# mikwieczorek/centroids-reid

Hardware: AMD Instinct MI355X
Metric: train_images_per_sec (higher is better)
Workload: dtype bf16; 1 GPU; ResNet50 256x128 CTL training step: fwd+bwd, centroid-triplet + center + xent, Adam + center SGD (BASELINE configs[1]); P=16, K=4, global_batch=64, num_classes=751, parallelism=single

## Files before the change

### centroids-reid_amd/_lib.py

```python
from __future__ import annotations

import ctypes as C
import os

import torch

_HERE = os.path.dirname(os.path.abspath(__file__))
LIB_PATH = os.environ.get("CREID_LIB_PATH") or os.path.join(_HERE, "lib", "libcreid_hip.so")

F32, BF16, F16 = 0, 1, 2
_DT = {torch.float32: F32, torch.bfloat16: BF16, torch.float16: F16}
BF16X3 = 3
EVAL_PRECISIONS = ("bf16x3",)
TRAIN_PRECISIONS = ("bf16x3",)

_lib = None

_p, _i64, _i32, _f32, _sz = C.c_void_p, C.c_int64, C.c_int32, C.c_float, C.c_size_t

SIGNATURES = {
    "creid_abi_version": (C.c_int, []),
    "creid_l2norm_rows": (C.c_int, [_p, _p, _p, _i64, _i64, C.c_int, _f32, _p]),
    "creid_row_sqnorm": (C.c_int, [_p, _p, _i64, _i64, C.c_int, _p]),
    "creid_sqdist_matrix": (C.c_int, [_p, _p, _p, _p, _i64, _i64, _i64, C.c_int, _p, _i64, _p]),
# ... 33 lines not shown
    "creid_ctl_heads_fused": (C.c_int, [_p, _p]),
    "creid_ctl_step_stats_rows": (C.c_int, [_p, _p, _i64, _i64, _i64, _p, _p, _p, _p]),
    "creid_center_loss_fwd_masked": (C.c_int, [_p, _p, _p, _p, _i64, _i64, _i64, _p, _p, _p]),
    "creid_center_loss_bwd_masked": (C.c_int, [_p, _p, _p, _p, _p, _i64, _i64, _p, _f32, _p, _p, _p]),
    "creid_xent_ls_masked": (C.c_int, [_p, _p, _p, _i64, _i64, _f32, _f32, _p, _p, _p, _p]),
    "creid_bn1d_fwd_masked": (C.c_int, [_p, _p, _i64, _i64, _p, _p, _p, _p, _f32, _f32, _p, _p, _p, _p]),
    "creid_bn1d_bwd_masked": (C.c_int, [_p, _p, _p, _i64, _i64, _p, _p, _p, _p, _p, _p, _p]),
    "creid_triplet_fwd": (C.c_int, [_p, _p, _p, _i64, _i64, _f32, _p, _p, _p, _p, _p, _p, _p, _p]),
    "creid_triplet_bwd": (C.c_int, [_p, _i64, _i64, _p, _p, _p, _p, _p, _p, _f32, _p, _p]),
    "creid_triplet_fwd_batched": (C.c_int, [_p, _p, _p, _i64, _i64, _i64, _f32, _p, _p, _p, _p, _p, _p, _p, _p]),
    "creid_triplet_bwd_batched": (C.c_int, [_p, _i64, _i64, _i64, _p, _p, _p, _p, _p, _p, _f32, _p, _p]),
    "creid_triplet_cosine_fwd": (C.c_int, [_p, _p, _p, _i64, _i64, _f32, _p, _p, _p, _p, _p, _p, _p, _p]),
    "creid_triplet_cosine_bwd": (C.c_int, [_p, _i64, _i64, _p, _p, _p, _p, _p, _p, _f32, _p, _p]),
    "creid_rownorm_fwd": (C.c_int, [_p, _i64, _i64, C.c_int, _f32, _p, _p, _p]),
    "creid_rownorm_bwd": (C.c_int, [_p, _p, _p, _i64, _i64, C.c_int, _f32, _p, _p]),
    "creid_hard_mine_from_dist": (C.c_int, [_p, _p, _i64, _p, _p, _p, _p, _p]),
    "creid_clamp_sqrt_inplace": (C.c_int, [_p, _i64, _f32, _p]),
    "creid_center_loss_fwd": (C.c_int, [_p, _p, _p, _i64, _i64, _i64, _p, _p, _p]),
    "creid_center_loss_bwd": (C.c_int, [_p, _p, _p, _p, _i64, _i64, _p, _f32, _p, _p, _p]),
    "creid_xent_ls": (C.c_int, [_p, _p, _i64, _i64, _f32, _f32, _p, _p, _p, _p]),
    "creid_bn1d_fwd": (C.c_int, [_p, _i64, _i64, _p, _p, _p, _p, C.c_int, _f32, _f32, _p, _p, _p, _p]),
    "creid_bn1d_bwd": (C.c_int, [_p, _p, _i64, _i64, _p, _p, _p, _p, _p, _p, _p]),
    "creid_gather_mean_rows": (C.c_int, [_p, _p, _p, _i64, _i64, _p, _p]),
    "creid_adam_step": (C.c_int, [_p, _p, _p, _p, _i64, _f32, _f32, _f32, _f32, _f32, _i64, _f32, _p]),
    "creid_adam_step_dev": (C.c_int, [_p, _p, _p, _p, _i64, _p, _f32, _f32, _f32, _f32, _f32, _p]),
    "creid_sgd_scaled_step": (C.c_int, [_p, _p, _i64, _f32, _f32, _p]),
    "creid_amp_scale": (C.c_int, [_p, _i64, _p, _p, _p]),
    "creid_amp_unscale_check": (C.c_int, [_p, _i64, _p, _p, _p]),
    "creid_amp_update": (C.c_int, [_p, _p, _f32, _f32, C.c_int32, _p]),
    "creid_adam_step_dev_amp": (C.c_int, [_p, _p, _p, _p, _i64, _p, _f32, _f32, _f32, _f32, _f32, _p, _p]),
    "creid_sgd_scaled_step_amp": (C.c_int, [_p, _p, _i64, _f32, _f32, _p, _p]),
    "creid_conv2d_bn_partial_rows": (_i64, [_p]),
    "creid_igemm_halo_launches": (_i64, []),
    "creid_conv2d_fwd_nhwc": (C.c_int, [_p, _p, _p, _p, _p, C.c_int, _p]),
    "creid_conv2d_fwd_affine_nhwc": (C.c_int, [_p, _p, _p, _p, _p, _p, C.c_int, C.c_int, _p]),
    "creid_conv1x1_bnrelu_fwd": (C.c_int, [_p, _p, _p, _i64, _i64, _i64, _p, _p, _p, _p, C.c_int, _p]),
    "creid_bn2d_fold_entry_bytes": (_i64, []),
    "creid_bn2d_fold_multi": (C.c_int, [_p, _i64, _p]),
    "creid_stem_conv_fwd_affine": (C.c_int, [_i64, _i64, _i64, _p, _p, _p, _p, C.c_int, C.c_int, _p]),
    "creid_stem_conv_pool_fwd_affine": (C.c_int, [_i64, _i64, _i64, _p, _p, _p, _p, C.c_int, C.c_int, _p]),
    "creid_bottleneck_c3_c1_fwd_affine": (C.c_int, [_i64, _i64, _i64, _i64, _p, _p, _p, _p, _p, _p, _p, _p, C.c_int, _p]),
    "creid_bottleneck_c3_c1_fwd_stats": (C.c_int, [_i64, _i64, _i64, _i64, _p, _p, _p, _p, _p, _p, _p, _p, C.c_int, _p]),
    "creid_conv2d_dgrad_nhwc": (C.c_int, [_p, _p, _p, _p, _p, C.c_int, _p]),
    "creid_conv2d_wgrad_workspace_bytes": (_sz, [_p, C.c_int]),
    "creid_conv2d_wgrad_nhwc": (C.c_int, [_p, _p, _p, _p, C.c_int, _p, _sz, C.c_int, _p]),
    "creid_conv2d_wgrad_partials": (C.c_int, [_p, _p, _p, _p, _sz, C.c_int, _p]),
    "creid_conv2d_wgrad_partials_bnfin": (C.c_int, [_p, _p, _p, _p, _sz, C.c_int, _p, _i64, _i64, _i64, _p, _p, _p, _p, _p, _p, _p]),
    "creid_conv2d_wgrad_reduce": (C.c_int, [_p, _p, C.c_int, _p, _sz, C.c_int, _p]),
    "creid_bn2d_bwd_finalize_wred": (C.c_int, [_p, _i64, _i64, _i64, _p, _p, _p, _p, _p, _p, _p, _p, C.c_int, _p, _sz, C.c_int, _p]),
    "creid_conv2d_wgrad_reduce_job": (C.c_int, [_p, _p, C.c_int, _p, _sz, C.c_int, _p]),
    "creid_conv2d_dgrad_x3_nhwc": (C.c_int, [_p, _p, _p, _p, _p, _p]),
    "creid_conv2d_wgrad_x3_workspace_bytes": (_sz, [_p]),
    "creid_conv2d_wgrad_x3_nhwc": (C.c_int, [_p, _p, _p, _p, C.c_int, _p, _sz, _p]),
    "creid_conv2d_wgrad_x3_partials": (C.c_int, [_p, _p, _p, _p, _sz, _p]),
    "creid_weight_prep_x3_train_multi": (C.c_int, [_p, _p, _i64, _i64, _p]),
    "creid_stem_conv_fwd": (C.c_int, [_i64, _i64, _i64, _p, _p, _p, _p, C.c_int, _p]),
    "creid_stem_conv_wgrad_workspace_bytes": (_sz, [_i64, _i64, _i64, C.c_int]),
    "creid_stem_conv_wgrad": (C.c_int, [_i64, _i64, _i64, _p, _p, _p, C.c_int, _p, _sz, C.c_int, _p]),
    "creid_image_to_nhwc4_pad": (C.c_int, [_p, _i64, _i64, _i64, C.c_int, _p, _p]),
    "creid_augment_u8": (C.c_int, [_p, _p, _i64, _i64, _i64, _i64] + [C.c_float] * 9 + [C.c_int32, C.c_int32, _p, _p]),
    "creid_resize_u8": (C.c_int, [_p, _i64, _p, _p, _p, _i64, _p, _i64, _i64, _i64, _p, _p]),
    "creid_weight_prep": (C.c_int, [_p, _i64, _i64, _i64, _i64, C.c_int, _p, _p, _p]),
    "creid_weight_prep_entry_bytes": (_i64, []),
    "creid_weight_prep_multi": (C.c_int, [_p, _p, _i64, _i64, C.c_int, _p]),
    "creid_stem_weight_prep": (C.c_int, [_p, C.c_int, _p, _p]),
    "creid_bn2d_finalize": (C.c_int, [_p, _i64, _i64, _i64, _p, _p, C.c_int, _f32, _f32, _p, _p, _p, _p, _p, _p]),
# ... 125 lines not shown
```

### centroids-reid_amd/csrc/bn_fin.hpp

```cpp
#pragma once
#include "common.hpp"

struct BnBwdFinJob {
  const float* partial;
  int rows, C;
  float inv_count;
  const float* mean;
  const float* invstd;
  const float* gamma;
  float* sums;
  float* dgamma;
  float* dbeta;
  int nblocks;
  int cw;
};

template <int NT, int CW>
__device__ __forceinline__ void bn_bwd_finalize_block_cw(const BnBwdFinJob& j, int block, void* lds) {
  constexpr int RG = NT / CW, NW = NT / 64;
  double* red = reinterpret_cast<double*>(lds);
  const int tid = threadIdx.x, cl = tid % CW, rg = tid / CW;
  const int c = block * CW + cl, C = j.C;
  double s1 = 0.0, s2 = 0.0;
  if (c < C) {
    int r = rg;
    for (; r + 3 * RG < j.rows; r += 4 * RG) {
      const float a0 = j.partial[((int64_t)r * 2) * C + c], b0 = j.partial[((int64_t)r * 2 + 1) * C + c];
      const float a1 = j.partial[((int64_t)(r + RG) * 2) * C + c], b1 = j.partial[((int64_t)(r + RG) * 2 + 1) * C + c];
      const float a2 = j.partial[((int64_t)(r + 2 * RG) * 2) * C + c], b2 = j.partial[((int64_t)(r + 2 * RG) * 2 + 1) * C + c];
      const float a3 = j.partial[((int64_t)(r + 3 * RG) * 2) * C + c], b3 = j.partial[((int64_t)(r + 3 * RG) * 2 + 1) * C + c];
      s1 += ((double)a0 + (double)a1) + ((double)a2 + (double)a3);
      s2 += ((double)b0 + (double)b1) + ((double)b2 + (double)b3);
    }
    for (; r < j.rows; r += RG) {
      s1 += (double)j.partial[((int64_t)r * 2) * C + c];
      s2 += (double)j.partial[((int64_t)r * 2 + 1) * C + c];
    }
  }
#pragma unroll
  for (int o = CW; o < 64; o <<= 1) { s1 += __shfl_xor(s1, o, 64); s2 += __shfl_xor(s2, o, 64); }
  if ((tid & 63) < CW) { red[((tid >> 6) * 2 + 0) * CW + cl] = s1; red[((tid >> 6) * 2 + 1) * CW + cl] = s2; }
  float p_mu = 0.f, p_is = 0.f, p_g = 1.f, p_db = 0.f, p_dg = 0.f;
  if (rg == 0 && c < C) {
    p_mu = j.mean[c]; p_is = j.invstd[c];
    if (j.gamma) p_g = j.gamma[c];
    if (j.dbeta) p_db = j.dbeta[c];
    if (j.dgamma) p_dg = j.dgamma[c];
  }
  __syncthreads();
  if (rg == 0 && c < C) {
    s1 = 0.0; s2 = 0.0;
#pragma unroll
    for (int q = 0; q < NW; ++q) { s1 += red[(q * 2 + 0) * CW + cl]; s2 += red[(q * 2 + 1) * CW + cl]; }
    const float invM = j.inv_count;
    const float mu = p_mu, is = p_is, k1 = p_g * is;
    const float a1 = (float)s1 * invM, a2 = (float)s2 * invM;
    j.sums[c] = k1;
    j.sums[C + c] = -k1 * is * a2;
    j.sums[2 * C + c] = -k1 * a1 + k1 * is * a2 * mu;
    if (j.dbeta) j.dbeta[c] = p_db + (float)s1;
    if (j.dgamma) j.dgamma[c] = p_dg + (float)s2;
  }
}

template <int NT>
__device__ __forceinline__ void bn_bwd_finalize_block(const BnBwdFinJob& j, int block, void* lds) {
  if (j.cw == 4) bn_bwd_finalize_block_cw<NT, 4>(j, block, lds);
  else bn_bwd_finalize_block_cw<NT, 16>(j, block, lds);
}

static inline void bn_bwd_fin_shape(BnBwdFinJob& j) {
  j.cw = (j.C <= 256 && j.rows >= 512) ? 4 : 16;
  j.nblocks = (j.C + j.cw - 1) / j.cw;
}
```

### centroids-reid_amd/csrc/conv_wgrad.hip

```cpp
#include "conv_common.hpp"
#include "wgrad_reduce.hpp"
#include "bn_fin.hpp"
#include "tune.hpp"
#include <stdlib.h>

namespace {
constexpr int WKS = 64;
constexpr int WKF = 16;
}

template <int OFF_HI>
__device__ __forceinline__ void tr_load4(const unsigned short* p, s16x4& f0lo, s16x4& f0hi, s16x4& f1lo, s16x4& f1hi) {
  const unsigned addr = (unsigned)(uintptr_t)p;
  asm volatile(
      "ds_read_b64_tr_b16 %0, %4\n\t"
      "ds_read_b64_tr_b16 %1, %4 offset:%5\n\t"
      "ds_read_b64_tr_b16 %2, %4 offset:64\n\t"
      "ds_read_b64_tr_b16 %3, %4 offset:%6"
      : "=&v"(f0lo), "=&v"(f0hi), "=&v"(f1lo), "=&v"(f1hi)
      : "v"(addr), "i"(OFF_HI), "i"(OFF_HI + 64)
      : "memory");
}
__device__ __forceinline__ void tr_wait8(s16x4& a, s16x4& b, s16x4& c, s16x4& d, s16x4& e, s16x4& f, s16x4& g, s16x4& h) {
  asm volatile("s_waitcnt lgkmcnt(0)" : "+v"(a), "+v"(b), "+v"(c), "+v"(d), "+v"(e), "+v"(f), "+v"(g), "+v"(h)::"memory");
}

template <int NW>
__device__ __forceinline__ void tr_wait8_n(s16x4& a, s16x4& b, s16x4& c, s16x4& d, s16x4& e, s16x4& f, s16x4& g, s16x4& h) {
  asm volatile("s_waitcnt lgkmcnt(%8)" : "+v"(a), "+v"(b), "+v"(c), "+v"(d), "+v"(e), "+v"(f), "+v"(g), "+v"(h) : "n"(NW) : "memory");
}

template <int NW, int IM, int JN>
__device__ __forceinline__ void tr_wait_set(s16x4 (&al)[IM], s16x4 (&ah)[IM], s16x4 (&bl)[JN], s16x4 (&bh)[JN]) {
  if constexpr (IM == 2 && JN == 2)
    asm volatile("s_waitcnt lgkmcnt(%8)" : "+v"(al[0]), "+v"(ah[0]), "+v"(al[1]), "+v"(ah[1]), "+v"(bl[0]), "+v"(bh[0]), "+v"(bl[1]), "+v"(bh[1]) : "n"(NW) : "memory");
  else if constexpr (IM == 2 && JN == 1)
    asm volatile("s_waitcnt lgkmcnt(%6)" : "+v"(al[0]), "+v"(ah[0]), "+v"(al[1]), "+v"(ah[1]), "+v"(bl[0]), "+v"(bh[0]) : "n"(NW) : "memory");
// ... 382 lines not shown
    float* ex = reinterpret_cast<float*>(smem_all);
    const int t256 = tid & 255;
    if (kg == 1) {
#pragma unroll
      for (int i = 0; i < IM; ++i)
#pragma unroll
        for (int j = 0; j < JN; ++j)
#pragma unroll
          for (int r = 0; r < 16; ++r) ex[((i * JN + j) * 16 + r) * 256 + t256] = acc[i][j][r];
    }
    __syncthreads();
    if (kg == 1) return;
#pragma unroll
    for (int i = 0; i < IM; ++i)
#pragma unroll
      for (int j = 0; j < JN; ++j)
#pragma unroll
        for (int r = 0; r < 16; ++r) acc[i][j][r] += ex[((i * JN + j) * 16 + r) * 256 + t256];
  }
  const int l31 = lane & 31, kh = lane >> 5;
  float* wsp = ws + (int64_t)split * NCO * g.K;
#pragma unroll
  for (int i = 0; i < IM; ++i)
#pragma unroll
    for (int j = 0; j < JN; ++j)
#pragma unroll
      for (int r = 0; r < 16; ++r) {
        const int co = co0 + wm * (TM / 2) + i * 32 + (r & 3) + 8 * (r >> 2) + 4 * kh;
        const int kc = k0 + wn * (TN / 2) + j * 32 + l31;
        wsp[(int64_t)co * g.K + kc] = acc[i][j][r];
      }
}

template <int TM, int TN>
__global__ __launch_bounds__(256) void wgrad_f32_kernel(IGemmGeom g, const float* __restrict__ dy,
                                                        const float* __restrict__ x, int NCO, float* __restrict__ ws,
                                                        int tiles_k, int m_per_split) {
  constexpr int IM = TM / 64, JN = TN / 64;
  constexpr int CA = TM / 4, CB = TN / 4;
  constexpr int RA = 256 / CA, RB = 256 / CB;
  constexpr int NA = (WKF + RA - 1) / RA, NBL = (WKF + RB - 1) / RB;
  __shared__ __attribute__((aligned(16))) float Ad[WKF][TM];
  __shared__ __attribute__((aligned(16))) float Bx[WKF][TN];
  const int tid = threadIdx.x, lane = tid & 63, wave = tid >> 6;
  const int wm = wave >> 1, wn = wave & 1;
  const int tile = blockIdx.x, split = blockIdx.y;
  const int tile_co = tile / tiles_k, tile_k = tile - tile_co * tiles_k;
  const int co0 = tile_co * TM, k0 = tile_k * TN;
  const int m_begin = split * m_per_split, m_end = min(g.M, m_begin + m_per_split);
  const int span_mask = (1 << g.log2span) - 1;
  const int a_ch = tid % CA, a_row = tid / CA;
  const int b_ch = tid % CB, b_row = tid / CB;
  const int kcol = k0 + 4 * b_ch;
  const int tap = kcol >> g.log2span, cc = kcol & span_mask;
  const int tr = tap / g.kw, ts = tap - tr * g.kw;
  float4 ra[NA], rb[NBL];
  auto gload = [&](int mb) {
#pragma unroll
    for (int i = 0; i < NA; ++i) {
      const int pr = a_row + RA * i, m = mb + pr;
      ra[i] = (pr < WKF && m < m_end) ? *reinterpret_cast<const float4*>(dy + (int64_t)m * NCO + co0 + 4 * a_ch)
                                      : make_float4(0.f, 0.f, 0.f, 0.f);
    }
#pragma unroll
    for (int i = 0; i < NBL; ++i) {
      const int pr = b_row + RB * i, m = mb + pr;
// ... 230 lines not shown
  for (int e = 0; e < 4; ++e) {
    const int kc = kc0 + e;
    const int tap = kc >> log2span, within = kc & span_mask;
    const int r = tap / kw_taps, s = tap % kw_taps + within / cpitch, c = within % cpitch;
    if (r < kh && s < kw && c < cin) {
      float* dst = dw_oihw + (((int64_t)co * cin + c) * kh + r) * kw + s;
      *dst = accumulate ? *dst + v[e] : v[e];
    }
  }
}

__global__ __launch_bounds__(256) void wgrad_reduce_taps_kernel(const float* __restrict__ ws, int splits, int NCO, int K,
                                                                int cin, int taps, float* __restrict__ dw_oihw,
                                                                int accumulate) {
  extern __shared__ float tr_lds[];
  const int co = blockIdx.x;
  const int64_t total = (int64_t)NCO * K;
  const float* src = ws + (int64_t)co * K;
  for (int e = threadIdx.x; e < K; e += 256) {
    float a0 = 0.f, a1 = 0.f;
    int sp = 0;
    for (; sp + 1 < splits; sp += 2) { a0 += src[(int64_t)sp * total + e]; a1 += src[(int64_t)(sp + 1) * total + e]; }
    if (sp < splits) a0 += src[(int64_t)sp * total + e];
    const int tap = e / cin, c = e - tap * cin;
    tr_lds[c * taps + tap] = a0 + a1;
  }
  __syncthreads();
  float* dst = dw_oihw + (int64_t)co * K;
  for (int e = threadIdx.x; e < K; e += 256) dst[e] = accumulate ? dst[e] + tr_lds[e] : tr_lds[e];
}

static int ilog2x(int64_t v) { int l = 0; while ((1LL << l) < v) ++l; return ((1LL << l) == v) ? l : -1; }

struct WgradPlan { int tm, tn, tiles, tiles_k, splits, m_per_split, xcd, stages, ws, kg; };

static WgradPlan plan_wgrad(int M, int NCO, int K, int dtype, int stride = 1) {
  static const int target = [] { const char* e = getenv("CREID_WGRAD_TARGET_WGS"); int v = e ? atoi(e) : 0; return v > 0 ? v : 512; }();
  static const int max_splits_pref = [] { const char* e = getenv("CREID_WGRAD_MAX_SPLITS"); int v = e ? atoi(e) : 0; return v > 0 ? v : (1 << 30); }();
  const int ks = creid_is16(dtype) ? WKS : WKF;
  const int cand[3][2] = {{128, 128}, {128, 64}, {64, 64}};
  WgradPlan p;
  p.stages = 0; p.ws = 0; p.kg = 0;
  TunePlan tp;
  const bool have_plan = creid_is16(dtype) && creid_tune_lookup(CREID_TUNE_WGRAD, M, NCO, K, stride << 1, tp);
  if (have_plan && !((tp.p0 == 64 || tp.p0 == 128) && (tp.p1 == 64 || tp.p1 == 128) && NCO % tp.p0 == 0 && K % tp.p1 == 0 && tp.p2 >= 1))
    creid_tune_declined(CREID_TUNE_WGRAD, M, NCO, K, stride << 1);
  else if (have_plan) {
    p.tm = tp.p0; p.tn = tp.p1;
    p.stages = (tp.p2 >> 16) & 15; p.ws = (tp.p2 >> 20) & 1; p.kg = (tp.p2 >> 21) & 1;
    tp.p2 &= 0xffff;
    p.tiles_k = K / p.tn;
    p.tiles = (NCO / p.tm) * p.tiles_k;
    int splits = tp.p2;
    const int max_splits = (M + ks - 1) / ks;
    if (splits > max_splits) splits = max_splits;
    p.m_per_split = ((M + splits - 1) / splits + ks - 1) / ks * ks;
    p.splits = (M + p.m_per_split - 1) / p.m_per_split;
    static const int xcd_mode = [] { const char* e = getenv("CREID_WGRAD_XCD"); return e ? atoi(e) : 1; }();
    p.xcd = (xcd_mode && p.splits >= 8) ? 1 : 0;
    return p;
  }
  for (int ci = 0; ci < 3; ++ci) {
    int tm = cand[ci][0], tn = cand[ci][1];
    if (NCO % tm != 0) tm = 64;
    if (K % tn != 0) tn = 64;
    p.tm = tm; p.tn = tn;
    p.tiles_k = K / tn;
    p.tiles = (NCO / tm) * p.tiles_k;
    int splits = (target + p.tiles - 1) / p.tiles;
    static const int xcd_mode = [] { const char* e = getenv("CREID_WGRAD_XCD"); return e ? atoi(e) : 1; }();
    p.xcd = 0;
    if (xcd_mode && creid_is16(dtype)) {
      if (splits >= 8) { splits = (splits + 4) / 8 * 8; p.xcd = 1; }
      else if (xcd_mode >= 2) { splits = splits >= 6 ? 8 : (splits >= 3 ? 4 : splits); p.xcd = 1; }
    }
    const int max_splits = (M + 4 * ks - 1) / (4 * ks);
    if (splits > max_splits) splits = max_splits;
    if (splits < 1) splits = 1;
    p.m_per_split = ((M + splits - 1) / splits + ks - 1) / ks * ks;
    p.splits = (M + p.m_per_split - 1) / p.m_per_split;
    if (p.xcd && p.splits < 8 && (8 % p.splits) != 0) p.xcd = 0;
    if (p.splits <= max_splits_pref) break;
  }
  return p;
}

__global__ __launch_bounds__(256) void bn_bwd_finalize_job_kernel(BnBwdFinJob j) {
  __shared__ __attribute__((aligned(16))) double fin_lds[4 * 2 * 16];
  bn_bwd_finalize_block<256>(j, (int)blockIdx.x, fin_lds);
}

template <int TM, int TN>
static bool launch_wgrad_t(const IGemmGeom& g, const void* dy, const void* x, int NCO, float* ws, const WgradPlan& p,
                           int dtype, hipStream_t s, const BnBwdFinJob* fin_in = nullptr) {
  dim3 grid((unsigned)p.tiles, (unsigned)p.splits), block(256);
  const bool xcd_on = p.xcd != 0;
  const int xt = xcd_on ? p.tiles : 0;
  const int share = p.splits >= 8 ? 1 : 8 / p.splits;
  BnBwdFinJob fin{};
  if (fin_in && xcd_on) fin = *fin_in;
  const unsigned nf8 = fin.partial ? (unsigned)((fin.nblocks + 7) & ~7) : 0u;
  const dim3 grid_x((p.splits >= 8 ? (unsigned)(p.tiles * ((p.splits + 7) / 8) * 8) : (unsigned)(8 * ((p.tiles + share - 1) / share))) + nf8);
  const dim3 grid_dma = xcd_on ? grid_x : grid;
  static const int use_dma = [] { const char* e = getenv("CREID_WGRAD_DMA"); return e ? atoi(e) : 1; }();
#ifdef CREID_ABL_BUILD
  static const int wg_abl = creid_ablation_env("CREID_WGRAD_ABL");
#else
  const int wg_abl = 0;
#endif
  static const int stages_env = [] { const char* e = getenv("CREID_WGRAD_STAGES"); int v = e ? atoi(e) : 0; return (v >= 2 && v <= 4) ? v : 2; }();
  static const int stem_dma = [] { const char* e = getenv("CREID_STEM_DMA"); return e ? atoi(e) : 1; }();
  const bool stem_geom = g.log2span == 5 && !g.check_bounds && g.kw == 1 && g.stride == 2 && g.pad == 0 && stem_dma;
  if (creid_is16(dtype) && use_dma && ((1 << g.log2span) >= TN || stem_geom)) {
    static const int use_ws_env = [] { const char* e = getenv("CREID_WGRAD_WS"); return e ? atoi(e) : 0; }();
    const int use_ws = p.ws ? 1 : use_ws_env;
    const int stages = (p.stages >= 2 && p.stages <= 4) ? p.stages : stages_env;
    static const int kg_env = [] { const char* e = getenv("CREID_WGRAD_KG"); return e ? atoi(e) : 0; }();
// ... 6 lines not shown
                           (const unsigned short*)x, NCO, ws, p.tiles_k, p.m_per_split, xt, p.splits, fin, wg_abl);               \
      else                                                                                                                        \
        hipLaunchKernelGGL((wgrad_bf16_dma_kernel<TM, TN, NS_, WS_, KG_, Bf16T>), grid_dma, BLOCK_, 0, s, g, (const unsigned short*)dy, \
                           (const unsigned short*)x, NCO, ws, p.tiles_k, p.m_per_split, xt, p.splits, fin, wg_abl);               \
    } while (0)
    if (kg2 && stages >= 3 && kg3_fits) {
      if constexpr (kg3_fits) CREID_WG_LAUNCH(3, false, 2, dim3(512));
    } else if (kg2) CREID_WG_LAUNCH(2, false, 2, dim3(512));
    else if (use_ws && !stem_geom) CREID_WG_LAUNCH(2, true, 1, dim3(512));
    else if (stages == 2) CREID_WG_LAUNCH(2, false, 1, block);
    else if (stages == 3) CREID_WG_LAUNCH(3, false, 1, block);
    else CREID_WG_LAUNCH(4, false, 1, block);
#undef CREID_WG_LAUNCH
    return fin.partial != nullptr;
  }
  else if (dtype == CREID_F16) return false;
  else if (dtype == CREID_BF16)
    hipLaunchKernelGGL((wgrad_bf16_kernel<TM, TN>), grid, block, 0, s, g, (const unsigned short*)dy,
                       (const unsigned short*)x, NCO, ws, p.tiles_k, p.m_per_split);
  else
    hipLaunchKernelGGL((wgrad_f32_kernel<TM, TN>), grid, block, 0, s, g, (const float*)dy, (const float*)x, NCO, ws,
                       p.tiles_k, p.m_per_split);
  return false;
}

static int run_wgrad(const IGemmGeom& g, const void* dy, const void* x, int NCO, float* dw, int kw_taps, int cpitch,
                     int cin, int kh, int kw, int accumulate, void* ws, size_t ws_bytes, int dtype, hipStream_t s,
                     int phases = 3, const BnBwdFinJob* fin = nullptr) {
  if (!creid_is16(dtype) && dtype != CREID_F32) return CREID_E_DTYPE;
  if (dtype == CREID_F16) {
    static const int dma_on = [] { const char* e = getenv("CREID_WGRAD_DMA"); return e ? atoi(e) : 1; }();
    if (!dma_on) return CREID_E_DTYPE;
  }
  const WgradPlan p = plan_wgrad(g.M, NCO, g.K, dtype, g.stride);
  if (dtype == CREID_F16 && (phases & 1)) {
    static const int stem_dma = [] { const char* e = getenv("CREID_STEM_DMA"); return e ? atoi(e) : 1; }();
    const bool stem_geom = g.log2span == 5 && !g.check_bounds && g.kw == 1 && g.stride == 2 && g.pad == 0 && stem_dma;
    if (!((1 << g.log2span) >= p.tn || stem_geom)) return CREID_E_SHAPE;
  }
  const size_t need = (size_t)p.splits * NCO * g.K * sizeof(float);
  if (ws_bytes < need) return CREID_E_WS;
  if (phases & 1) {
    bool carried;
    if (p.tm == 128 && p.tn == 128) carried = launch_wgrad_t<128, 128>(g, dy, x, NCO, (float*)ws, p, dtype, s, fin);
    else if (p.tm == 128 && p.tn == 64) carried = launch_wgrad_t<128, 64>(g, dy, x, NCO, (float*)ws, p, dtype, s, fin);
    else if (p.tm == 64 && p.tn == 128) carried = launch_wgrad_t<64, 128>(g, dy, x, NCO, (float*)ws, p, dtype, s, fin);
    else carried = launch_wgrad_t<64, 64>(g, dy, x, NCO, (float*)ws, p, dtype, s, fin);
    if (fin && !carried)
      hipLaunchKernelGGL(bn_bwd_finalize_job_kernel, dim3((unsigned)fin->nblocks), dim3(256), 0, s, *fin);
  }
  if (!(phases & 2)) return (int)hipGetLastError();
  if (kh * kw == 9 && cpitch == cin && (1 << g.log2span) == cin && kw_taps == kw && p.splits <= 16 &&
      (size_t)g.K * sizeof(float) <= 48 * 1024) {
    hipLaunchKernelGGL(wgrad_reduce_taps_kernel, dim3((unsigned)NCO), dim3(256), (size_t)g.K * sizeof(float), s,
                       (const float*)ws, p.splits, NCO, g.K, cin, 9, dw, accumulate);
    return (int)hipGetLastError();
  }
  const int64_t total4 = (int64_t)NCO * g.K / 4;
#define CREID_WRED(SL_)                                                                                              \
  hipLaunchKernelGGL(wgrad_reduce_kernel<SL_>, dim3((unsigned)((total4 + 256 / SL_ - 1) / (256 / SL_))), dim3(256), 0, s, \
                     (const float*)ws, p.splits, NCO, g.K, g.log2span, kw_taps, cpitch, cin, kh, kw, dw, accumulate)
  if (p.splits <= 8) CREID_WRED(1);
  else if (p.splits <= 32) CREID_WRED(4);
  else if (p.splits <= 128) CREID_WRED(16);
  else CREID_WRED(64);
#undef CREID_WRED
  return (int)hipGetLastError();
}

__global__ __launch_bounds__(512) void wgrad_reduce_job_kernel(WRedJob j) {
  extern __shared__ __attribute__((aligned(16))) float wred_lds[];
  wgrad_reduce_block<512>(j, (int)blockIdx.x, wred_lds);
}

int wgrad_reduce_job_launch(const WRedJob& j, hipStream_t s) {
  hipLaunchKernelGGL(wgrad_reduce_job_kernel, dim3((unsigned)j.nblocks), dim3(512), (size_t)(4 * 512 + j.K) * sizeof(float), s, j);
  return (int)hipGetLastError();
}

bool wgrad_make_reduce_job(const creid_conv_desc* d, int dtype, const void* ws, size_t ws_bytes, float* dw, int accumulate,
                           WRedJob& j) {
  if (!d || !ws || !dw) return false;
  const int M = (int)(d->batch * d->out_h * d->out_w), K = (int)(d->kh * d->kw * d->in_c), NCO = (int)d->out_c;
  const WgradPlan p = plan_wgrad(M, NCO, K, dtype, d->stride);
  if (ws_bytes < (size_t)p.splits * NCO * K * sizeof(float)) return false;
  const bool ok = wred_make_job(j, (const float*)ws, dw, p.splits, NCO, K, (int)d->in_c, d->kh, d->kw, accumulate);
  static const int dry = creid_ablation_env("CREID_WRED_DRY");
  if (ok && dry) { j.K = 0; j.splits = 0; }
  return ok;
}

extern "C" {

size_t creid_conv2d_wgrad_workspace_bytes(const creid_conv_desc* d, int dtype) {
  if (!d) return 0;
  const int M = (int)(d->batch * d->out_h * d->out_w), K = (int)(d->kh * d->kw * d->in_c);
  const WgradPlan p = plan_wgrad(M, (int)d->out_c, K, dtype, d->stride);
  return (size_t)p.splits * d->out_c * K * sizeof(float);
}

static int conv_wgrad_phases(const creid_conv_desc* d, const void* x, const void* dy, float* dw_oihw, int accumulate,
                             void* ws, size_t ws_bytes, int dtype, void* stream, int phases, const BnBwdFinJob* fin = nullptr);

int creid_conv2d_wgrad_nhwc(const creid_conv_desc* d, const void* x, const void* dy, float* dw_oihw, int accumulate,
                            void* ws, size_t ws_bytes, int dtype, void* stream) {
  CREID_CHECK_ARG(x && dy && dw_oihw);
  return conv_wgrad_phases(d, x, dy, dw_oihw, accumulate, ws, ws_bytes, dtype, stream, 3);
}

int creid_conv2d_wgrad_partials(const creid_conv_desc* d, const void* x, const void* dy, void* ws, size_t ws_bytes,
                                int dtype, void* stream) {
  CREID_CHECK_ARG(x && dy);
  return conv_wgrad_phases(d, x, dy, nullptr, 0, ws, ws_bytes, dtype, stream, 1);
}

int creid_conv2d_wgrad_partials_bnfin(const creid_conv_desc* d, const void* x, const void* dy, void* ws, size_t ws_bytes,
                                      int dtype, const float* bn_partial, int64_t bn_rows, int64_t bn_C, int64_t bn_count,
                                      const float* bn_mean, const float* bn_invstd, const float* bn_gamma, float* bn_sums,
                                      float* bn_dgamma, float* bn_dbeta, void* stream) {
  CREID_CHECK_ARG(x && dy && bn_partial && bn_mean && bn_invstd && bn_sums && bn_rows > 0 && bn_C > 0 && bn_count > 0);
  BnBwdFinJob fin{bn_partial, (int)bn_rows, (int)bn_C, (float)(1.0 / (double)bn_count), bn_mean, bn_invstd, bn_gamma, bn_sums,
                  bn_dgamma, bn_dbeta, 0, 16};
  bn_bwd_fin_shape(fin);
  return conv_wgrad_phases(d, x, dy, nullptr, 0, ws, ws_bytes, dtype, stream, 1, &fin);
}

int creid_conv2d_wgrad_reduce(const creid_conv_desc* d, float* dw_oihw, int accumulate, const void* ws, size_t ws_bytes,
                              int dtype, void* stream) {
  CREID_CHECK_ARG(dw_oihw);
  return conv_wgrad_phases(d, nullptr, nullptr, dw_oihw, accumulate, const_cast<void*>(ws), ws_bytes, dtype, stream, 2);
}

__global__ __launch_bounds__(512) void wred_bnfin_kernel(WRedJob j, BnBwdFinJob fin) {
  extern __shared__ __attribute__((aligned(16))) float wredfin_lds[];
  const int nf8 = fin.partial ? ((fin.nblocks + 7) & ~7) : 0;
// ... 98 lines not shown
```

### include/creid.h

```cpp
#ifndef CREID_H
#define CREID_H

#include <stddef.h>
#include <stdint.h>

#ifdef __cplusplus
extern "C" {
#endif

#define CREID_ABI_VERSION 1

enum { CREID_F32 = 0, CREID_BF16 = 1, CREID_F16 = 2, CREID_BF16X3 = 3 };
enum { CREID_E_ARG = -1, CREID_E_DTYPE = -2, CREID_E_WS = -3, CREID_E_SHAPE = -4 };

int creid_abi_version(void);


int creid_l2norm_rows(const float* x, void* y, float* sqnorm, int64_t rows, int64_t D,
                      int out_dtype, float eps, void* stream);

int creid_row_sqnorm(const void* x, float* out, int64_t rows, int64_t D, int dtype, void* stream);

int creid_sqdist_matrix(const void* q, const void* g, const float* qq, const float* gg,
                        int64_t m, int64_t n, int64_t D, int dtype, float* out, int64_t ldo,
// ... 197 lines not shown
int creid_gather_mean_rows(const float* emb, const int64_t* order, const int64_t* offsets,
                           int64_t n_seg, int64_t D, float* out, void* stream);


int creid_adam_step(float* p, const float* g, float* m, float* v, int64_t n, float lr, float beta1,
                    float beta2, float eps, float weight_decay, int64_t step, float grad_scale,
                    void* stream);
int creid_adam_step_dev(float* p, const float* g, float* m, float* v, int64_t n, float* hyper_dev,
                        float beta1, float beta2, float eps, float weight_decay, float grad_scale,
                        void* stream);
int creid_sgd_scaled_step(float* p, float* g, int64_t n, float lr, float grad_mul, void* stream);

int creid_amp_scale(const float* x, int64_t n, const float* amp_state, float* y, void* stream);
int creid_amp_unscale_check(float* g, int64_t n, const float* amp_state, int32_t* amp_flags, void* stream);
int creid_amp_update(float* amp_state, int32_t* amp_flags, float growth_factor, float backoff_factor, int32_t growth_interval,
                     void* stream);
int creid_adam_step_dev_amp(float* p, const float* g, float* m, float* v, int64_t n, float* hyper_dev, float beta1, float beta2,
                            float eps, float weight_decay, float grad_scale, const int32_t* skip_flag, void* stream);
int creid_sgd_scaled_step_amp(float* p, float* g, int64_t n, float lr, float grad_mul, const int32_t* skip_flag, void* stream);


int creid_gemm_f32(const float* A, int64_t sam, int64_t sak, const float* B, int64_t sbk, int64_t sbn,
                   float* C, int64_t ldc, int64_t M, int64_t N, int64_t K, float alpha, float beta,
                   int32_t split_k, void* stream);


typedef struct {
  int64_t batch, in_h, in_w, in_c, out_h, out_w, out_c;
  int32_t kh, kw, stride, pad;
} creid_conv_desc;

int64_t creid_conv2d_bn_partial_rows(const creid_conv_desc* d);
int64_t creid_igemm_halo_launches(void);
int creid_conv2d_fwd_nhwc(const creid_conv_desc* d, const void* x, const void* w_krsc, void* y,
                          float* bn_partial, int dtype, void* stream);
int creid_conv2d_fwd_affine_nhwc(const creid_conv_desc* d, const void* x, const void* w_krsc, void* y,
                                 const float* scale_shift, const void* residual, int relu, int dtype, void* stream);
int creid_conv1x1_bnrelu_fwd(const void* x_raw, const float* scale_shift, const void* w_krsc, int64_t M, int64_t K, int64_t N,
                             void* y, float* bn_partial, void* a_out, uint8_t* mask_out, int dtype, void* stream);
int64_t creid_bn2d_fold_entry_bytes(void);
int creid_bn2d_fold_multi(const void* table_dev, int64_t n_entries, void* stream);
int creid_conv2d_dgrad_nhwc(const creid_conv_desc* d, const void* dy, const void* w_crsk, void* dx,
                            const void* add_src, int dtype, void* stream);
int creid_conv2d_dgrad_x3_nhwc(const creid_conv_desc* d, const void* dy, const void* w2_crsk, void* dx, const void* add_src,
                               void* stream);
int creid_conv2d_dgrad_bnred_nhwc(const creid_conv_desc* d, const void* dy, const void* w_crsk, void* dx,
                                  const void* add_src, const void* bn_x, const void* bn_act,
                                  const float* bn_mean, const float* bn_invstd, float* bn_partial,
                                  int64_t bn_stat_image_rows, int add_src_stride, int dtype, void* stream);

int creid_conv2d_dgrad_fused_nhwc(const creid_conv_desc* d, const void* dy, const void* w_crsk, void* dx,
                                  const void* add_src, int add_src_stride, const uint8_t* add_mask, const void* bn_x,
                                  const void* bn_act, const uint8_t* bn_mask, const float* bn_mean, const float* bn_invstd,
                                  float* bn_partial, int64_t bn_stat_image_rows, const creid_conv_desc* wred_desc, float* wred_dw,
                                  int wred_accumulate, const void* wred_ws, size_t wred_ws_bytes, int dtype,
                                  void* stream);
size_t creid_conv2d_wgrad_workspace_bytes(const creid_conv_desc* d, int dtype);
int creid_conv2d_wgrad_nhwc(const creid_conv_desc* d, const void* x, const void* dy, float* dw_oihw,
                            int accumulate, void* ws, size_t ws_bytes, int dtype, void* stream);
int creid_conv2d_wgrad_partials(const creid_conv_desc* d, const void* x, const void* dy, void* ws,
                                size_t ws_bytes, int dtype, void* stream);
int creid_bn2d_bwd_finalize_wred(const float* bn_partial, int64_t bn_rows, int64_t bn_C, int64_t bn_count,
                                 const float* bn_mean, const float* bn_invstd, const float* bn_gamma, float* bn_sums,
                                 float* bn_dgamma, float* bn_dbeta, const creid_conv_desc* wred_desc, float* wred_dw,
                                 int wred_accumulate, const void* wred_ws, size_t wred_ws_bytes, int dtype, void* stream);
int creid_conv2d_wgrad_reduce_job(const creid_conv_desc* d, float* dw_oihw, int accumulate, const void* ws,
// ... 115 lines not shown
```

Measured before the change: 10840 images/s.

## Add halo-tile taps wgrad kernel for 3x3 stride-1 bf16 convolutions

```diff
diff --git a/centroids-reid_amd/_lib.py b/centroids-reid_amd/_lib.py
--- a/centroids-reid_amd/_lib.py
+++ b/centroids-reid_amd/_lib.py
@@ -89,6 +89,7 @@
     "creid_sgd_scaled_step_amp": (C.c_int, [_p, _p, _i64, _f32, _f32, _p, _p]),
     "creid_conv2d_bn_partial_rows": (_i64, [_p]),
     "creid_igemm_halo_launches": (_i64, []),
+    "creid_wgrad_taps_launches": (_i64, []),
     "creid_conv2d_fwd_nhwc": (C.c_int, [_p, _p, _p, _p, _p, C.c_int, _p]),
     "creid_conv2d_fwd_affine_nhwc": (C.c_int, [_p, _p, _p, _p, _p, _p, C.c_int, C.c_int, _p]),
     "creid_conv1x1_bnrelu_fwd": (C.c_int, [_p, _p, _p, _i64, _i64, _i64, _p, _p, _p, _p, C.c_int, _p]),
diff --git a/centroids-reid_amd/csrc/bn_fin.hpp b/centroids-reid_amd/csrc/bn_fin.hpp
--- a/centroids-reid_amd/csrc/bn_fin.hpp
+++ b/centroids-reid_amd/csrc/bn_fin.hpp
@@ -16,7 +16,8 @@
 };
 
 template <int NT, int CW>
-__device__ __forceinline__ void bn_bwd_finalize_block_cw(const BnBwdFinJob& j, int block, void* lds) {
+__device__ __forceinline__ void bn_bwd_finalize_block_cw(const BnBwdFinJob& j, int block, void* lds, bool active = true) {
+  if (!active) { __syncthreads(); return; }
   constexpr int RG = NT / CW, NW = NT / 64;
   double* red = reinterpret_cast<double*>(lds);
   const int tid = threadIdx.x, cl = tid % CW, rg = tid / CW;
@@ -64,9 +65,9 @@
 }
 
 template <int NT>
-__device__ __forceinline__ void bn_bwd_finalize_block(const BnBwdFinJob& j, int block, void* lds) {
-  if (j.cw == 4) bn_bwd_finalize_block_cw<NT, 4>(j, block, lds);
-  else bn_bwd_finalize_block_cw<NT, 16>(j, block, lds);
+__device__ __forceinline__ void bn_bwd_finalize_block(const BnBwdFinJob& j, int block, void* lds, bool active = true) {
+  if (j.cw == 4) bn_bwd_finalize_block_cw<NT, 4>(j, block, lds, active);
+  else bn_bwd_finalize_block_cw<NT, 16>(j, block, lds, active);
 }
 
 static inline void bn_bwd_fin_shape(BnBwdFinJob& j) {
diff --git a/centroids-reid_amd/csrc/conv_wgrad.hip b/centroids-reid_amd/csrc/conv_wgrad.hip
--- a/centroids-reid_amd/csrc/conv_wgrad.hip
+++ b/centroids-reid_amd/csrc/conv_wgrad.hip
@@ -3,6 +3,7 @@
 #include "bn_fin.hpp"
 #include "tune.hpp"
 #include <stdlib.h>
+#include <atomic>
 
 namespace {
 constexpr int WKS = 64;
@@ -451,6 +452,193 @@
       }
 }
 
+constexpr int TPK = 128;
+
+template <int OW>
+struct TapsGeom {
+  static constexpr int ROWS = TPK / OW, HP = OW + 2, NSLOT = (ROWS + 2) * HP;
+  static constexpr int NIH = (NSLOT + 63) / 64;
+  static constexpr int TILE_A = TPK * 64, STAGE = TILE_A + NIH * 64 * 64;
+  static constexpr int slice_slot(int kk) { return kk * 16 + 2 * ((kk * 16) / OW); }
+};
+
+template <int NW>
+__device__ __forceinline__ void tr_wait_unit(s16x4& al, s16x4& ah, s16x4 (&bl)[3], s16x4 (&bh)[3]) {
+  asm volatile("s_waitcnt lgkmcnt(%8)" : "+v"(al), "+v"(ah), "+v"(bl[0]), "+v"(bh[0]), "+v"(bl[1]), "+v"(bh[1]), "+v"(bl[2]), "+v"(bh[2]) : "n"(NW) : "memory");
+}
+
+template <int OW, int U>
+__device__ __forceinline__ void taps_load_unit(unsigned fa, const unsigned (&fb)[9], unsigned sb, s16x4 (&al)[2], s16x4 (&ah)[2],
+                                               s16x4 (&bl)[2][3], s16x4 (&bh)[2][3]) {
+  constexpr int KK = U / 3, G = U % 3, S = TapsGeom<OW>::slice_slot(KK), FLIP = ((S >> 1) & 1) * 64;
+  if constexpr (G == 0) tr_load2<KK * 16 * 128, (KK * 16 + 4) * 128>(fa + sb, al[KK & 1], ah[KK & 1]);
+#pragma unroll
+  for (int j = 0; j < 3; ++j) tr_load2<S * 128, (S + 4) * 128>((fb[3 * G + j] ^ (unsigned)FLIP) + sb, bl[U & 1][j], bh[U & 1][j]);
+}
+
+template <int OW, typename ET, int U>
+__device__ __forceinline__ void taps_unit(unsigned fa, const unsigned (&fb)[9], unsigned sb, s16x4 (&al)[2], s16x4 (&ah)[2],
+                                          s16x4 (&bl)[2][3], s16x4 (&bh)[2][3], f32x16 (&acc)[9]) {
+  constexpr int NU = 3 * (TPK / 32), KK = U / 3, G = U % 3;
+  if constexpr (U + 1 < NU) {
+    taps_load_unit<OW, U + 1>(fa, fb, sb, al, ah, bl, bh);
+    tr_wait_unit<((U + 1) % 3 == 0) ? 8 : 6>(al[KK & 1], ah[KK & 1], bl[U & 1], bh[U & 1]);
+  } else {
+    tr_wait_unit<0>(al[KK & 1], ah[KK & 1], bl[U & 1], bh[U & 1]);
+  }
+  __builtin_amdgcn_sched_barrier(0);
+  const s16x8 a = __builtin_shufflevector(al[KK & 1], ah[KK & 1], 0, 1, 2, 3, 4, 5, 6, 7);
+#pragma unroll
+  for (int j = 0; j < 3; ++j) {
+    const s16x8 b = __builtin_shufflevector(bl[U & 1][j], bh[U & 1][j], 0, 1, 2, 3, 4, 5, 6, 7);
+    acc[3 * G + j] = ET::mfma(a, b, acc[3 * G + j]);
+  }
+  __builtin_amdgcn_sched_barrier(0);
+  if constexpr (U + 1 < NU) taps_unit<OW, ET, U + 1>(fa, fb, sb, al, ah, bl, bh, acc);
+}
+
+template <int OW, typename ET>
+__global__ __launch_bounds__(512, 2) void wgrad_bf16_taps_kernel(const unsigned short* __restrict__ dy, const unsigned short* __restrict__ x,
+                                                                  int M, int OH, int CIN, int NCO, float* __restrict__ ws, int tiles,
+                                                                  int tiles_ci, int splits, int m_per_split, BnBwdFinJob fin) {
+  using G = TapsGeom<OW>;
+  constexpr int NS = 3, NIA = TPK / 64, NIH = G::NIH, LPT = NIA + NIH, STAGE = G::STAGE;
+  static_assert(NS * STAGE * 2 <= 160 * 1024 && (NS - 2) * LPT <= 63 && (G::slice_slot(7) + 4) * 128 < 65536, "LDS ring / vmcnt / ds offset");
+  static_assert(((G::slice_slot(4) >> 1) & 1) == 0 && G::slice_slot(5) - G::slice_slot(1) == G::slice_slot(4) &&
+                G::slice_slot(6) - G::slice_slot(2) == G::slice_slot(4) && G::slice_slot(7) - G::slice_slot(3) == G::slice_slot(4), "k-groups");
+  static_assert(5 * 16 * 256 * 4 <= NS * STAGE * 2, "accumulator exchange");
+  __shared__ __attribute__((aligned(1024))) unsigned short smem[NS * STAGE];
+  const int tid = threadIdx.x, lane = tid & 63, wave = tid >> 6;
+  const int kg = wave >> 2, wm = (wave >> 1) & 1, wn = wave & 1;
+  int bid0 = (int)blockIdx.x;
+  if (fin.partial) {
+    const int nf8 = (fin.nblocks + 7) & ~7;
+    if (bid0 < nf8) {
+      if (bid0 < fin.nblocks) bn_bwd_finalize_block<256>(fin, bid0, smem, tid < 256);
+      return;
+    }
+    bid0 -= nf8;
+  }
+  int tile, split;
+  if (splits >= 8 || (8 % splits) != 0) {
+    const int j = bid0 >> 3, ls = j / tiles;
+    tile = j - ls * tiles;
+    split = (bid0 & 7) + 8 * ls;
+    if (split >= splits) return;
+  } else {
+    const int x8 = bid0 & 7, share = 8 / splits;
+    split = x8 % splits;
+    tile = x8 / splits + share * (bid0 >> 3);
+    if (tile >= tiles) return;
+  }
+  const int tile_co = tile / tiles_ci, tile_ci = tile - tile_co * tiles_ci;
+  const int co0 = tile_co * 64, ci0 = tile_ci * 64;
+  const int m_begin = split * m_per_split, m_end = min(M, m_begin + m_per_split);
+  const int nt = (m_end - m_begin) / TPK;
+  const unsigned short* zpage = reinterpret_cast<const unsigned short*>(g_wgrad_zero_page);
+
+  const int dr = lane >> 3, dq = lane & 7;
+  const unsigned short* pa[NIA];
+#pragma unroll
+  for (int i = 0; i < NIA; ++i) {
+    const int row = (i * 8 + wave) * 8 + dr, key = (row >> 1) & 1;
+    pa[i] = dy + (int64_t)(m_begin + row) * NCO + co0 + (((((dq >> 2) ^ key) << 2) + (dq & 3)) << 3);
+  }
+  int hoff[NIH], hrow[NIH];
+#pragma unroll
+  for (int i = 0; i < NIH; ++i) {
+    const int t = (i * 8 + wave) * 8 + dr, hr = t / G::HP, hx = t - hr * G::HP, key = (t >> 1) & 1;
+    const bool xok = t < G::NSLOT && hx >= 1 && hx <= OW;
+    hrow[i] = xok ? hr - 1 : (1 << 20);
+    hoff[i] = ((hr - 1) * OW + hx - 1) * CIN + ci0 + (((((dq >> 2) ^ key) << 2) + (dq & 3)) << 3);
+  }
+  const unsigned short* xs = x + (int64_t)m_begin * CIN;
+  int oy0 = (m_begin % (OH * OW)) / OW;
+  typedef const void __attribute__((address_space(1)))* gptr_t;
+  typedef void __attribute__((address_space(3)))* lptr_t;
+  auto issue = [&](int buf) {
+    unsigned short* la = smem + buf * STAGE + wave * 512;
+    unsigned short* lh = la + G::TILE_A;
+#pragma unroll
+    for (int i = 0; i < NIA; ++i) {
+      __builtin_amdgcn_global_load_lds((gptr_t)pa[i], (lptr_t)(la + i * 4096), 16, 0, 0);
+      pa[i] += (int64_t)TPK * NCO;
+    }
+#pragma unroll
+    for (int i = 0; i < NIH; ++i) {
+      const unsigned short* p = ((unsigned)(oy0 + hrow[i]) < (unsigned)OH) ? xs + hoff[i] : zpage;
+      __builtin_amdgcn_global_load_lds((gptr_t)p, (lptr_t)(lh + i * 4096), 16, 0, 0);
+    }
+    xs += (int64_t)TPK * CIN;
+    oy0 += G::ROWS;
+    if (oy0 >= OH) oy0 = 0;
+  };
+
+  f32x16 acc[9];
+#pragma unroll
+  for (int t = 0; t < 9; ++t)
+#pragma unroll
+    for (int r = 0; r < 16; ++r) acc[t][r] = 0.f;
+
+  const int li = lane & 15;
+  const int t_row = 8 * (lane >> 5) + (li >> 2), t_col = 16 * ((lane >> 4) & 1) + 4 * (li & 3);
+  const unsigned lds0 = (unsigned)(uintptr_t)smem;
+  const int cola = wm * 32 + t_col, colb = wn * 32 + t_col;
+  const unsigned fa = lds0 + 2u * (unsigned)((kg * 64 + t_row) * 64 + (((cola >> 5) ^ ((t_row >> 1) & 1)) << 5) + (cola & 31));
+  const int slot0 = t_row + 2 * (t_row / OW) + kg * G::slice_slot(4);
+  unsigned fb[9];
+#pragma unroll
+  for (int t = 0; t < 9; ++t) {
+    const int slot = slot0 + (t / 3) * G::HP + (t % 3);
+    fb[t] = lds0 + 2u * (unsigned)(G::TILE_A + slot * 64 + (((colb >> 5) ^ ((slot >> 1) & 1)) << 5) + (colb & 31));
+  }
+  auto compute = [&](unsigned sb) {
+    s16x4 al[2], ah[2], bl[2][3], bh[2][3];
+    taps_load_unit<OW, 0>(fa, fb, sb, al, ah, bl, bh);
+    taps_unit<OW, ET, 0>(fa, fb, sb, al, ah, bl, bh, acc);
+  };
+#pragma unroll
+  for (int p = 0; p < NS - 1; ++p)
+    if (p < nt) issue(p);
+  int buf = 0;
+  for (int t = 0; t < nt; ++t) {
+    const int younger = min(nt - 1 - t, NS - 2);
+    if (younger == 1) wg_wait_vm<LPT>(); else wg_wait_vm<0>();
+    asm volatile("s_barrier" ::: "memory");
+    if (t + NS - 1 < nt) issue(buf == 0 ? NS - 1 : buf - 1);
+    compute((unsigned)(buf * STAGE * 2));
+    buf = (buf + 1 == NS) ? 0 : buf + 1;
+  }
+  {
+    float* ex = reinterpret_cast<float*>(smem);
+    const int t256 = tid & 255;
+#pragma unroll
+    for (int t0 = 0; t0 < 9; t0 += 5) {
+      __syncthreads();
+      if (kg == 1) {
+#pragma unroll
+        for (int t = t0; t < (t0 == 0 ? 5 : 9); ++t)
+#pragma unroll
+          for (int r = 0; r < 16; ++r) ex[((t - t0) * 16 + r) * 256 + t256] = acc[t][r];
+      }
+      __syncthreads();
+      if (kg == 0) {
+#pragma unroll
+        for (int t = t0; t < (t0 == 0 ? 5 : 9); ++t)
+#pragma unroll
+          for (int r = 0; r < 16; ++r) acc[t][r] += ex[((t - t0) * 16 + r) * 256 + t256];
+      }
+    }
+    if (kg == 1) return;
+  }
+  const int l31 = lane & 31, kh = lane >> 5, K = 9 * CIN;
+  float* wsp = ws + ((int64_t)split * NCO + co0 + wm * 32 + 4 * kh) * K + ci0 + wn * 32 + l31;
+#pragma unroll
+  for (int t = 0; t < 9; ++t)
+#pragma unroll
+    for (int r = 0; r < 16; ++r) wsp[(int64_t)((r & 3) + 8 * (r >> 2)) * K + t * CIN] = acc[t][r];
+}
+
 template <int TM, int TN>
 __global__ __launch_bounds__(256) void wgrad_f32_kernel(IGemmGeom g, const float* __restrict__ dy,
                                                         const float* __restrict__ x, int NCO, float* __restrict__ ws,
@@ -747,7 +935,7 @@
 
 static int ilog2x(int64_t v) { int l = 0; while ((1LL << l) < v) ++l; return ((1LL << l) == v) ? l : -1; }
 
-struct WgradPlan { int tm, tn, tiles, tiles_k, splits, m_per_split, xcd, stages, ws, kg; };
+struct WgradPlan { int tm, tn, tiles, tiles_k, splits, m_per_split, xcd, stages, ws, kg, taps; };
 
 static WgradPlan plan_wgrad(int M, int NCO, int K, int dtype, int stride = 1) {
   static const int target = [] { const char* e = getenv("CREID_WGRAD_TARGET_WGS"); int v = e ? atoi(e) : 0; return v > 0 ? v : 512; }();
@@ -755,7 +943,7 @@
   const int ks = creid_is16(dtype) ? WKS : WKF;
   const int cand[3][2] = {{128, 128}, {128, 64}, {64, 64}};
   WgradPlan p;
-  p.stages = 0; p.ws = 0; p.kg = 0;
+  p.stages = 0; p.ws = 0; p.kg = 0; p.taps = 0;
   TunePlan tp;
   const bool have_plan = creid_is16(dtype) && creid_tune_lookup(CREID_TUNE_WGRAD, M, NCO, K, stride << 1, tp);
   if (have_plan && !((tp.p0 == 64 || tp.p0 == 128) && (tp.p1 == 64 || tp.p1 == 128) && NCO % tp.p0 == 0 && K % tp.p1 == 0 && tp.p2 >= 1))
@@ -798,6 +986,61 @@
     if (p.splits <= max_splits_pref) break;
   }
   return p;
+}
+
+struct WgradShape { int kh, kw, pad, cin, OH, OW, SH, SW; };
+
+static WgradShape wgrad_shape_of(const creid_conv_desc* d) {
+  return WgradShape{d->kh, d->kw, d->pad, (int)d->in_c, (int)d->out_h, (int)d->out_w, (int)d->in_h, (int)d->in_w};
+}
+
+static std::atomic<int64_t> g_taps_launches{0};
+
+static bool wgrad_taps_covers(int M, int NCO, int dtype, int stride, const WgradShape& sh) {
+  if (!creid_is16(dtype) || sh.kh != 3 || sh.kw != 3 || stride != 1 || sh.pad != 1) return false;
+  if (sh.cin != 64 && sh.cin != 128 && sh.cin != 256 && sh.cin != 512) return false;
+  if (NCO <= 0 || NCO % 64 != 0 || sh.SH != sh.OH || sh.SW != sh.OW) return false;
+  if (sh.OW != 8 && sh.OW != 16 && sh.OW != 32) return false;
+  return (sh.OH * sh.OW) % TPK == 0 && M > 0 && M % (sh.OH * sh.OW) == 0;
+}
+
+static WgradPlan plan_wgrad_route(int M, int NCO, int K, int dtype, int stride, const WgradShape& sh) {
+  WgradPlan p = plan_wgrad(M, NCO, K, dtype, stride);
+  const char* e = CREID_KNOB_ENV("CREID_WGRAD_TAPS");
+  if ((e && atoi(e) == 0) || !wgrad_taps_covers(M, NCO, dtype, stride, sh)) return p;
+  p.taps = 1; p.tm = 64; p.tn = 64; p.stages = 3; p.ws = 0; p.kg = 0; p.xcd = 1;
+  p.tiles_k = sh.cin / 64;
+  p.tiles = (NCO / 64) * p.tiles_k;
+  const int steps = M / TPK;
+  const char* we = CREID_KNOB_ENV("CREID_WGRAD_TAPS_WGS");
+  const int target = (we && atoi(we) > 0) ? atoi(we) : (p.tiles <= 4 ? 192 : 256);
+  int splits = (target + p.tiles / 2) / p.tiles;
+  if (splits > steps) splits = steps;
+  if (splits < 1) splits = 1;
+  const int per = (steps + splits - 1) / splits;
+  p.m_per_split = per * TPK;
+  p.splits = (steps + per - 1) / per;
+  return p;
+}
+
+static bool launch_wgrad_taps(const IGemmGeom& g, const void* dy, const void* x, int NCO, float* ws, const WgradPlan& p, int dtype,
+                              hipStream_t s, const BnBwdFinJob* fin_in) {
+  BnBwdFinJob fin{};
+  if (fin_in) fin = *fin_in;
+  const unsigned nf8 = fin.partial ? (unsigned)((fin.nblocks + 7) & ~7) : 0u;
+  const bool ranged = p.splits >= 8 || (8 % p.splits) != 0;
+  const int share = ranged ? 1 : 8 / p.splits;
+  const unsigned nwg = ranged ? (unsigned)(p.tiles * ((p.splits + 7) / 8) * 8) : (unsigned)(8 * ((p.tiles + share - 1) / share));
+  const int cin = 1 << g.log2span;
+#define CREID_WT_LAUNCH(OW_, ET_)                                                                                          \
+  hipLaunchKernelGGL((wgrad_bf16_taps_kernel<OW_, ET_>), dim3(nwg + nf8), dim3(512), 0, s, (const unsigned short*)dy,      \
+                     (const unsigned short*)x, g.M, g.OH, cin, NCO, ws, p.tiles, p.tiles_k, p.splits, p.m_per_split, fin)
+#define CREID_WT_OW(OW_) do { if (dtype == CREID_F16) CREID_WT_LAUNCH(OW_, F16T); else CREID_WT_LAUNCH(OW_, Bf16T); } while (0)
+  if (g.OW == 8) CREID_WT_OW(8); else if (g.OW == 16) CREID_WT_OW(16); else CREID_WT_OW(32);
+#undef CREID_WT_OW
+#undef CREID_WT_LAUNCH
+  g_taps_launches.fetch_add(1, std::memory_order_relaxed);
+  return fin.partial != nullptr;
 }
 
 __global__ __launch_bounds__(256) void bn_bwd_finalize_job_kernel(BnBwdFinJob j) {
@@ -870,8 +1113,9 @@
     static const int dma_on = [] { const char* e = getenv("CREID_WGRAD_DMA"); return e ? atoi(e) : 1; }();
     if (!dma_on) return CREID_E_DTYPE;
   }
-  const WgradPlan p = plan_wgrad(g.M, NCO, g.K, dtype, g.stride);
-  if (dtype == CREID_F16 && (phases & 1)) {
+  const WgradShape shp{(cpitch == cin && kw_taps == kw && g.check_bounds && (1 << g.log2span) == cin) ? kh : 0, kw, g.pad, cin, g.OH, g.OW, g.SH, g.SW};
+  const WgradPlan p = plan_wgrad_route(g.M, NCO, g.K, dtype, g.stride, shp);
+  if (dtype == CREID_F16 && (phases & 1) && !p.taps) {
     static const int stem_dma = [] { const char* e = getenv("CREID_STEM_DMA"); return e ? atoi(e) : 1; }();
     const bool stem_geom = g.log2span == 5 && !g.check_bounds && g.kw == 1 && g.stride == 2 && g.pad == 0 && stem_dma;
     if (!((1 << g.log2span) >= p.tn || stem_geom)) return CREID_E_SHAPE;
@@ -880,7 +1124,8 @@
   if (ws_bytes < need) return CREID_E_WS;
   if (phases & 1) {
     bool carried;
-    if (p.tm == 128 && p.tn == 128) carried = launch_wgrad_t<128, 128>(g, dy, x, NCO, (float*)ws, p, dtype, s, fin);
+    if (p.taps) carried = launch_wgrad_taps(g, dy, x, NCO, (float*)ws, p, dtype, s, fin);
+    else if (p.tm == 128 && p.tn == 128) carried = launch_wgrad_t<128, 128>(g, dy, x, NCO, (float*)ws, p, dtype, s, fin);
     else if (p.tm == 128 && p.tn == 64) carried = launch_wgrad_t<128, 64>(g, dy, x, NCO, (float*)ws, p, dtype, s, fin);
     else if (p.tm == 64 && p.tn == 128) carried = launch_wgrad_t<64, 128>(g, dy, x, NCO, (float*)ws, p, dtype, s, fin);
     else carried = launch_wgrad_t<64, 64>(g, dy, x, NCO, (float*)ws, p, dtype, s, fin);
@@ -920,7 +1165,7 @@
                            WRedJob& j) {
   if (!d || !ws || !dw) return false;
   const int M = (int)(d->batch * d->out_h * d->out_w), K = (int)(d->kh * d->kw * d->in_c), NCO = (int)d->out_c;
-  const WgradPlan p = plan_wgrad(M, NCO, K, dtype, d->stride);
+  const WgradPlan p = plan_wgrad_route(M, NCO, K, dtype, d->stride, wgrad_shape_of(d));
   if (ws_bytes < (size_t)p.splits * NCO * K * sizeof(float)) return false;
   const bool ok = wred_make_job(j, (const float*)ws, dw, p.splits, NCO, K, (int)d->in_c, d->kh, d->kw, accumulate);
   static const int dry = creid_ablation_env("CREID_WRED_DRY");
@@ -933,12 +1178,14 @@
 size_t creid_conv2d_wgrad_workspace_bytes(const creid_conv_desc* d, int dtype) {
   if (!d) return 0;
   const int M = (int)(d->batch * d->out_h * d->out_w), K = (int)(d->kh * d->kw * d->in_c);
-  const WgradPlan p = plan_wgrad(M, (int)d->out_c, K, dtype, d->stride);
+  const WgradPlan p = plan_wgrad_route(M, (int)d->out_c, K, dtype, d->stride, wgrad_shape_of(d));
   return (size_t)p.splits * d->out_c * K * sizeof(float);
 }
 
 static int conv_wgrad_phases(const creid_conv_desc* d, const void* x, const void* dy, float* dw_oihw, int accumulate,
                              void* ws, size_t ws_bytes, int dtype, void* stream, int phases, const BnBwdFinJob* fin = nullptr);
+
+int64_t creid_wgrad_taps_launches(void) { return (int64_t)g_taps_launches.load(std::memory_order_relaxed); }
 
 int creid_conv2d_wgrad_nhwc(const creid_conv_desc* d, const void* x, const void* dy, float* dw_oihw, int accumulate,
                             void* ws, size_t ws_bytes, int dtype, void* stream) {
diff --git a/include/creid.h b/include/creid.h
--- a/include/creid.h
+++ b/include/creid.h
@@ -253,6 +253,7 @@
 
 int64_t creid_conv2d_bn_partial_rows(const creid_conv_desc* d);
 int64_t creid_igemm_halo_launches(void);
+int64_t creid_wgrad_taps_launches(void);
 int creid_conv2d_fwd_nhwc(const creid_conv_desc* d, const void* x, const void* w_krsc, void* y,
                           float* bn_partial, int dtype, void* stream);
 int creid_conv2d_fwd_affine_nhwc(const creid_conv_desc* d, const void* x, const void* w_krsc, void* y,
```

Measured after the change: 11010 images/s, median of 6. 1.5% higher.
